# bcgsc/RNA-Bloom

Hardware: AMD Instinct MI355X
Metric: k-mers/sec hashed+inserted into Bloom dBG (k=25, 50M 150bp reads) (higher is better)
Workload: dtype u64

## Files before the change

rna-bloom_amd/csrc/rb_capi.hip:

```cpp
#include <math.h>
#include <stdarg.h>
#include <stdlib.h>
#include <string.h>
#include <time.h>

#include <algorithm>
#include <new>
#include <vector>

#include <functional>
#include <string>
#include <thread>

#include <fcntl.h>
#include <unistd.h>
#include <zlib.h>

#include "rb_pipeline.hpp"

using namespace rb;

namespace {

__global__ void k_popcount_bits(const uint32_t *__restrict__ w, size_t n_words, unsigned long long *out) {
// ... 62 lines not shown

}

extern "C" {

int rb_version(void) { return 1; }
const char *rb_last_error(void) { return rb::last_error_text(); }

int rb_graph_create(const rb_graph_params *p, rb_graph **out) {
    rb_graph *g = nullptr;
    int rc = guarded([&] {
        RB_REQUIRE(p && out, "rb_graph_create: null argument");
        RB_REQUIRE(p->k >= 1 && p->k <= RB_MAX_K, "rb_graph_create: k=%d out of range [1,%d]", p->k, RB_MAX_K);
        RB_REQUIRE(p->dbgbf_bits > 0 && p->cbf_bytes > 0, "rb_graph_create: filter sizes must be positive");
        RB_REQUIRE(p->dbgbf_num_hash >= 1 && p->dbgbf_num_hash <= RB_MAX_HASH && p->cbf_num_hash >= 1 &&
                   p->cbf_num_hash <= RB_MAX_HASH, "rb_graph_create: numHash out of range [1,%d]", RB_MAX_HASH);
        if (p->use_read_paired_kmers)
            RB_REQUIRE(p->pkbf_bits > 0 && p->pkbf_num_hash >= 1 && p->pkbf_num_hash <= RB_MAX_HASH,
                       "rb_graph_create: pair filter parameters invalid");
        int ndev = 0;
        RB_HIP(hipGetDeviceCount(&ndev));
        RB_REQUIRE(p->device >= 0 && p->device < ndev, "rb_graph_create: device %d not present (%d devices)", p->device, ndev);
        RB_HIP(hipSetDevice(p->device));
        g = new rb_graph();
        g->p = *p;
        g->k = p->k;
        g->stranded = p->stranded != 0;
        g->H = std::max(p->dbgbf_num_hash, p->cbf_num_hash);
        g->max_batch_kmers = p->max_batch_kmers > 0 ? p->max_batch_kmers : ((int64_t)1 << 30);
        RB_REQUIRE(p->group_bits >= 0 && p->group_bits <= 64, "rb_graph_create: group_bits out of range [0,64]");
        if (p->group_bits) g->sort_begin_bit = 64 - p->group_bits;
        if (const char *e = getenv("RB_LIGHT_OPS")) g->light_ops = (uint32_t)std::max(1, atoi(e));
        if (const char *e = getenv("RB_SMALL_COMPONENT_OPS")) g->small_ops = (uint32_t)std::max(1, atoi(e));
        if (const char *e = getenv("RB_SORT_BEGIN_BIT")) g->sort_begin_bit = std::max(0, std::min(63, atoi(e)));
        RB_REQUIRE(g->max_batch_kmers <= ((int64_t)1 << 31), "rb_graph_create: max_batch_kmers above 2^31");
        if (const char *e = getenv("RB_CONSUMER_PRIORITY")) RB_HIP(hipStreamCreateWithPriority(&g->stream.s, hipStreamNonBlocking, atoi(e)));
        else RB_HIP(hipStreamCreateWithFlags(&g->stream.s, hipStreamNonBlocking));
        {
            int lo_p = 0, hi_p = 0;
            RB_HIP(hipDeviceGetStreamPriorityRange(&lo_p, &hi_p));
            int pr = hi_p;
            if (const char *e = getenv("RB_PRODUCER_PRIORITY")) pr = atoi(e);
            RB_HIP(hipStreamCreateWithPriority(&g->stream2.s, hipStreamNonBlocking, pr));
            RB_HIP(hipStreamCreateWithPriority(&g->stream3.s, hipStreamNonBlocking, pr));
        }
        RB_HIP(hipStreamCreateWithFlags(&g->pk_stream.s, hipStreamNonBlocking));
        RB_HIP(hipEventCreate(&g->ev0.e));
        RB_HIP(hipEventCreate(&g->ev1.e));
        RB_HIP(hipEventCreateWithFlags(&g->ev2.e, hipEventDisableTiming));
        RB_HIP(hipEventCreateWithFlags(&g->ev3.e, hipEventDisableTiming));
        alloc_bits(g->dbg, p->dbgbf_bits, p->dbgbf_num_hash, 0, p->dbgbf_bits);
        g->cbf_size = p->cbf_bytes; g->cbf_lo = 0; g->cbf_hi = p->cbf_bytes;
        g->cbf_alloc = (((size_t)p->cbf_bytes + 3) / 4 + 1) * 4;
        g->cbf_h = p->cbf_num_hash;
        g->cbf_mod = make_mod((uint64_t)p->cbf_bytes);
        g->cbf = static_cast<uint8_t *>(rb::alloc_best_placed(g->cbf_alloc, "cbf"));
        if (p->use_read_paired_kmers) { alloc_bits(g->rpk, p->pkbf_bits, p->pkbf_num_hash, 0, p->pkbf_bits); alloc_pair_seen(g->rpk); }
        {
            const char *e = getenv("RB_NPF");
            uint32_t l2 = log2_ceil((uint64_t)std::max<int64_t>(p->cbf_bytes / 64, 1));
            l2 = std::max(16u, std::min(28u, l2));
            if (e) l2 = (uint32_t)atoi(e);
            if (l2 >= 8 && l2 <= 30) {
                g->npf.reserve(sizeof(uint64_t) << l2);
                RB_HIP(hipMemset(g->npf.p, 0, sizeof(uint64_t) << l2));
                g->npf_log2 = l2;
// ... 813 lines not shown
```

rna-bloom_amd/csrc/rb_graph.hip:

```cpp
#include <math.h>
#include <stdarg.h>
#include <stdlib.h>
#include <string.h>
#include <time.h>

#include <algorithm>
#include <new>
#include <vector>

#include <functional>
#include <string>
#include <thread>

#include <fcntl.h>
#include <unistd.h>
#include <zlib.h>

#include "rb_pipeline.hpp"

using namespace rb;

namespace rb {
static thread_local char g_err[768] = "";
const char *last_error_text() { return g_err; }
// ... 482 lines not shown
    uint64_t idx[RB_MAX_HASH];
    bool conflict = (st & ST_FOREIGN) != 0;
    for (int j = 0; j < fv.cbf_h; ++j) {
        idx[j] = index_of(multi_hash(h0, (uint32_t)j, fv.kmul), fv.cbf_mod);
        if (n_foreign && !conflict) {
            const uint64_t b = slot_of(idx[j], csf_log2);
            if (!csf || ((csf[b >> 5] >> (uint32_t)(b & 31u)) & 1u)) conflict = table_find(cs, cs_log2, idx[j]) != nullptr;
        }
    }
    if (ops == 0) {
        for (int j = 0; j < fv.cbf_h; ++j) cbf_release(fv.cbf, idx[j]);
        return;
    }
    if (conflict) { status[d] = st | RUN_CONFLICT; return; }
    if (ops > LIGHT_OPS) { status[d] = st | RUN_HEAVY; return; }
    apply_light_run(fv, h0, occ_d, idx, cv_d, 0u, kfirst, krest, tz, start_d + m - ops, ops, mode);
}

__global__ void k_conf_release(FilterView fv, const uint64_t *__restrict__ uniq, const uint32_t *__restrict__ conf_kmers,
                               uint32_t n_conf) {
    uint32_t i = blockIdx.x * blockDim.x + threadIdx.x;
    if (i >= n_conf) return;
    const uint64_t h0 = uniq[conf_kmers[i]];
    for (int j = 0; j < fv.cbf_h; ++j) cbf_release(fv.cbf, index_of(multi_hash(h0, (uint32_t)j, fv.kmul), fv.cbf_mod));
}

__global__ void k_conf_offsets(const uint32_t *__restrict__ conf_kmers, const uint32_t *__restrict__ nops,
                               uint32_t n_conf, uint32_t *__restrict__ sizes) {
    uint32_t i = blockIdx.x * blockDim.x + threadIdx.x;
    if (i < n_conf) sizes[i] = nops[conf_kmers[i]];
    if (i == n_conf) sizes[i] = 0;
}
__global__ void k_label_init(FilterView fv, const uint64_t *__restrict__ uniq, const uint32_t *__restrict__ conf_kmers, uint32_t n_conf,
                             const Slot *ctable, uint32_t c_log2, uint32_t *__restrict__ label, uint32_t *__restrict__ lslot) {
    uint32_t i = blockIdx.x * blockDim.x + threadIdx.x;
    if (i >= n_conf) return;
    const uint32_t d = conf_kmers[i];
    label[d] = d;
    const uint64_t h0 = uniq[d];
    for (int j = 0; j < fv.cbf_h; ++j) {
        const Slot *sl = table_find(ctable, c_log2, index_of(multi_hash(h0, (uint32_t)j, fv.kmul), fv.cbf_mod));
        lslot[(size_t)i * fv.cbf_h + j] = sl ? (uint32_t)(sl - ctable) : CS_NONE;
    }
}
__global__ void k_label_round(int h, const uint32_t *__restrict__ conf_kmers, uint32_t n_conf, Slot *ctable, const uint32_t *__restrict__ lslot,
                              uint32_t *__restrict__ label, uint32_t *__restrict__ changed) {
    uint32_t i = blockIdx.x * blockDim.x + threadIdx.x;
    if (i >= n_conf) return;
    const uint32_t d = conf_kmers[i];
    const uint32_t l0 = __hip_atomic_load(&label[d], __ATOMIC_RELAXED, __HIP_MEMORY_SCOPE_AGENT);
    uint32_t l = l0, sl[RB_MAX_HASH];
    for (int j = 0; j < h; ++j) {
        sl[j] = lslot[(size_t)i * h + j];
        if (sl[j] == CS_NONE) continue;
        const uint32_t v = __hip_atomic_load(reinterpret_cast<const uint32_t *>(&ctable[sl[j]].val), __ATOMIC_RELAXED, __HIP_MEMORY_SCOPE_AGENT);
        l = v < l ? v : l;
    }
    const uint32_t up = __hip_atomic_load(&label[l], __ATOMIC_RELAXED, __HIP_MEMORY_SCOPE_AGENT);
    l = up < l ? up : l;
    bool moved = l != l0;
    if (moved) __hip_atomic_store(&label[d], l, __ATOMIC_RELAXED, __HIP_MEMORY_SCOPE_AGENT);
    for (int j = 0; j < h; ++j)
        if (sl[j] != CS_NONE && atomicMin(reinterpret_cast<uint32_t *>(&ctable[sl[j]].val), l) > l) moved = true;
    if (moved) *changed = 1u;
}
__global__ void k_conf_kmer_keys(const uint32_t *__restrict__ conf_kmers, const uint32_t *__restrict__ label,
                                 uint32_t n_conf, uint64_t *__restrict__ keys) {
    uint32_t i = blockIdx.x * blockDim.x + threadIdx.x;
    if (i < n_conf) { uint32_t d = conf_kmers[i]; keys[i] = ((uint64_t)label[d] << 32) | d; }
}
__global__ void k_conf_expand(const uint32_t *__restrict__ conf_kmers, const uint32_t *__restrict__ conf_off,
                              const uint32_t *__restrict__ counts, const uint32_t *__restrict__ starts,
                              const uint32_t *__restrict__ vals, const uint32_t *__restrict__ status,
                              const uint32_t *__restrict__ nops, const uint32_t *__restrict__ label, uint32_t n_conf,
                              uint64_t *__restrict__ op_key, uint32_t *__restrict__ op_val) {
    const uint32_t wave = (blockIdx.x * blockDim.x + threadIdx.x) >> 3, lane = threadIdx.x & 7u;
    if (wave >= n_conf) return;
    const uint32_t d = conf_kmers[wave];
    const uint32_t ops = nops[d], st = status[d];
    const uint64_t hi = (uint64_t)label[d] << 32;
    const uint32_t base = starts[d] + counts[d] - ops, out = conf_off[wave];
    for (uint32_t i = lane; i < ops; i += 8u) {
        op_key[out + i] = hi | vals[base + i];
        uint32_t kind = i == 0 ? (st >> 12) & 3u : (st >> 14) & 3u;
        op_val[out + i] = d | (kind << 30);
    }
}

__device__ __forceinline__ uint32_t lower_bound_u64(const uint64_t *a, uint32_t n, uint64_t key) {
    uint32_t lo = 0, hi = n;
    while (lo < hi) { uint32_t mid = (lo + hi) >> 1; if (a[mid] < key) lo = mid + 1; else hi = mid; }
    return lo;
}
__device__ void replay_serial(const FilterView &fv, const uint64_t *__restrict__ uniq, const uint64_t *__restrict__ op_key,
                              const uint32_t *__restrict__ op_val, uint32_t os, uint32_t oe) {
    uint64_t idx[RB_MAX_HASH];
    uint32_t c[RB_MAX_HASH], cur_d = 0xFFFFFFFFu;
    for (uint32_t i = os; i < oe; ++i) {
        const uint32_t v = (uint32_t)op_key[i];
        const uint32_t ov = op_val[i], d = ov & 0x3FFFFFFFu, kind = ov >> 30;
        if (d != cur_d) {
            const uint64_t h0 = uniq[d];
            for (int j = 0; j < fv.cbf_h; ++j) {
                idx[j] = index_of(multi_hash(h0, (uint32_t)j, fv.kmul), fv.cbf_mod);
                c[j] = *(volatile uint8_t *)&fv.cbf[idx[j]];
            }
            cur_d = d;
        }
        uint32_t c0[RB_MAX_HASH];
        for (int j = 0; j < fv.cbf_h; ++j) c0[j] = c[j];
        uint32_t mn = c[0];
        for (int j = 1; j < fv.cbf_h; ++j) mn = c[j] < mn ? c[j] : mn;
        cbf_step(c, fv.cbf_h, kind, (mn >= 16u && mn < 127u) ? occ_rnd(fv, v) : 0u);
        for (int j = 0; j < fv.cbf_h; ++j)
            if (c[j] != c0[j]) *(volatile uint8_t *)&fv.cbf[idx[j]] = (uint8_t)c[j];
    }
}
constexpr uint32_t MAX_COMPONENT_KMERS = 8;
__global__ void k_conf_replay_small(FilterView fv, const uint64_t *__restrict__ uniq, const uint64_t *__restrict__ kmer_keys,
                                    uint32_t n_conf, const uint64_t *__restrict__ op_key, const uint32_t *__restrict__ op_val,
                                    uint32_t n_ops, uint32_t *__restrict__ big_list, uint32_t *__restrict__ n_big, int store_cache,
                                    const uint32_t *__restrict__ starts, const uint32_t *__restrict__ vals, uint32_t small_ops) {
    uint32_t i = blockIdx.x * blockDim.x + threadIdx.x;
    if (i >= n_conf) return;
    const uint32_t lab = (uint32_t)(kmer_keys[i] >> 32);
    if (i > 0 && (uint32_t)(kmer_keys[i - 1] >> 32) == lab) return;
    const uint32_t os = lower_bound_u64(op_key, n_ops, (uint64_t)lab << 32);
    const uint32_t oe = lower_bound_u64(op_key, n_ops, ((uint64_t)lab + 1ull) << 32);
    if (oe - os > small_ops) { big_list[atomicAdd(n_big, 1u)] = i; return; }
    replay_serial(fv, uniq, op_key, op_val, os, oe);
    if (store_cache && cache_on(fv))
        for (uint32_t q = i; q < n_conf && (uint32_t)(kmer_keys[q] >> 32) == lab; ++q) {
            const uint32_t dq = (uint32_t)kmer_keys[q];
            const uint64_t h0 = uniq[dq];
            uint32_t mn = 255u;
            for (int j = 0; j < fv.cbf_h; ++j) {
                const uint32_t c = *(volatile uint8_t *)&fv.cbf[index_of(multi_hash(h0, (uint32_t)j, fv.kmul), fv.cbf_mod)];
                mn = c < mn ? c : mn;
            }
            if (mn >= 16u && mn < 128u) cache_store(fv, h0, vals[starts[dq]], cache_exp(mn));
        }
}
__global__ void __launch_bounds__(64) k_conf_replay_big(FilterView fv, const uint64_t *__restrict__ uniq,
                                    const uint64_t *__restrict__ kmer_keys, uint32_t n_conf,
                                    const uint64_t *__restrict__ op_key, const uint32_t *__restrict__ op_val, uint32_t n_ops,
                                    const uint32_t *__restrict__ big_list, const uint32_t *__restrict__ n_big,
                                    uint32_t *__restrict__ dbg, int store_cache,
                                    const uint32_t *__restrict__ starts, const uint32_t *__restrict__ vals) {
    __shared__ uint32_t s_drun[MAX_COMPONENT_KMERS];
    __shared__ uint64_t s_idx[MAX_COMPONENT_KMERS * RB_MAX_HASH];
    __shared__ uint32_t s_val[MAX_COMPONENT_KMERS * RB_MAX_HASH];
    __shared__ uint32_t s_val0[MAX_COMPONENT_KMERS * RB_MAX_HASH];
    __shared__ uint32_t s_slot[MAX_COMPONENT_KMERS][RB_MAX_HASH];
    __shared__ uint64_t s_h0[MAX_COMPONENT_KMERS];
    __shared__ uint32_t s_nu, s_nk;
    const uint32_t lane = threadIdx.x;
    const int H = fv.cbf_h;
    for (uint32_t bi = blockIdx.x; bi < *n_big; bi += gridDim.x) {
        const uint32_t i0 = big_list[bi];
        const uint32_t lab = (uint32_t)(kmer_keys[i0] >> 32);
        const uint32_t i1 = lower_bound_u64(kmer_keys, n_conf, ((uint64_t)lab + 1ull) << 32);
        const uint32_t os = lower_bound_u64(op_key, n_ops, (uint64_t)lab << 32);
        const uint32_t oe = lower_bound_u64(op_key, n_ops, ((uint64_t)lab + 1ull) << 32);
        __syncthreads();
        if (lane == 0) s_nk = 0;
        __syncthreads();
        bool overflow = false;
        for (uint32_t rb0 = i0; rb0 < i1 && !overflow; rb0 += 64u) {
            const bool have = rb0 + lane < i1;
            const uint32_t myd = have ? (uint32_t)kmer_keys[rb0 + lane] : 0u;
            const uint64_t h = have ? uniq[myd] : 0ull;
            unsigned long long pending = __ballot(have);
            while (pending) {
                const int leader = __ffsll((long long)pending) - 1;
                const uint64_t hl = __shfl(h, leader, 64);
                const uint32_t dl = __shfl(myd, leader, 64);
                pending &= ~__ballot(have && h == hl);
                uint32_t q = 0, nkc = s_nk;
                while (q < nkc && s_h0[q] != hl) ++q;
                if (q == nkc) {
                    if (nkc == MAX_COMPONENT_KMERS) { overflow = true; break; }
                    __syncthreads();
                    if (lane == 0) { s_h0[nkc] = hl; s_drun[nkc] = dl; s_nk = nkc + 1u; }
                    __syncthreads();
                }
            }
        }
        if (dbg && lane == 0) { atomicMax(&dbg[1], oe - os); atomicMax(&dbg[2], i1 - i0); atomicAdd(&dbg[3], oe - os); }
        if (overflow) {
            if (dbg && lane == 0) { atomicAdd(&dbg[0], 1u); atomicAdd(&dbg[4], oe - os); }
            if (lane == 0) replay_serial(fv, uniq, op_key, op_val, os, oe);
            continue;
        }
        const uint32_t nk = s_nk;
        __syncthreads();
        if (lane == 0) {
            uint32_t nu = 0;
            for (uint32_t q = 0; q < nk; ++q) {
                const uint64_t h0 = s_h0[q];
                for (int j = 0; j < H; ++j) {
                    const uint64_t idx = index_of(multi_hash(h0, (uint32_t)j, fv.kmul), fv.cbf_mod);
                    uint32_t u = 0;
                    while (u < nu && s_idx[u] != idx) ++u;
                    if (u == nu) { s_idx[u] = idx; s_val0[u] = s_val[u] = fv.cbf[idx]; ++nu; }
                    s_slot[q][j] = u;
                }
            }
            s_nu = nu;
        }
        __syncthreads();
        for (uint32_t base = os; base < oe; base += 64u) {
            const uint32_t i = base + lane;
            uint32_t q = 0, kind = 0, rnd = 0;
            const bool live = i < oe;
            if (live) {
                const uint32_t ov = op_val[i];
                const uint64_t h = uniq[ov & 0x3FFFFFFFu];
                kind = ov >> 30;
                while (q < nk && s_h0[q] != h) ++q;
                rnd = occ_rnd(fv, (uint32_t)op_key[i]);
            }
            uint32_t cursor = 0;
            while (cursor < 64u) {
                bool changes = false;
                if (live && lane >= cursor) {
                    uint32_t mn = s_val[s_slot[q][0]];
                    for (int j = 1; j < H; ++j) { uint32_t c = s_val[s_slot[q][j]]; mn = c < mn ? c : mn; }
                    const bool gate = !((kind == K_INC_IF_POS && mn == 0u) || (kind == K_INC_IF_ZERO && mn != 0u));
                    changes = gate && minifloat_inc(mn, rnd) != mn;
                }
                const unsigned long long win = __ballot(changes);
                if (!win) break;
                const uint32_t first = (uint32_t)__ffsll((long long)win) - 1u;
                if (lane == first) {
                    uint32_t mn = s_val[s_slot[q][0]];
                    for (int j = 1; j < H; ++j) { uint32_t c = s_val[s_slot[q][j]]; mn = c < mn ? c : mn; }
                    for (int j = 0; j < H; ++j) if (s_val[s_slot[q][j]] == mn) s_val[s_slot[q][j]] = mn + 1u;
                }
                __syncthreads();
                cursor = first + 1u;
            }
            __syncthreads();
        }
        if (lane < s_nu && s_val[lane] != s_val0[lane]) fv.cbf[s_idx[lane]] = (uint8_t)s_val[lane];
        if (store_cache && cache_on(fv) && lane < nk) {
            uint32_t mn = s_val[s_slot[lane][0]];
            for (int j = 1; j < H; ++j) { const uint32_t c = s_val[s_slot[lane][j]]; mn = c < mn ? c : mn; }
            if (mn >= 16u && mn < 128u) cache_store(fv, s_h0[lane], vals[starts[s_drun[lane]]], cache_exp(mn));
        }
        __syncthreads();
    }
}

__device__ __forceinline__ uint32_t next_unusable(const uint32_t *__restrict__ vw, uint32_t p, uint32_t L) {
    while (p < L) {
        const uint32_t w = ~vw[p >> 5] >> (p & 31u);
        if (w) { const uint32_t q = p + (uint32_t)__ffs((int)w) - 1u; return q < L ? q : L; }
        p = (p | 31u) + 1u;
    }
    return L;
}
template <int MODE, bool OUT>
__global__ void k_pairs_insert(const uint64_t *__restrict__ codes, const uint32_t *__restrict__ valid,
                               const uint32_t *__restrict__ word_read, const uint32_t *__restrict__ woff,
                               const uint32_t *__restrict__ len, int64_t w0, int64_t nw, int k, int dist,
                               uint32_t *bits, Mod mod, int num_hash, uint64_t kmul,
                               unsigned long long *__restrict__ n_pairs,
                               const uint32_t *__restrict__ chunk_off, uint64_t *__restrict__ out_idx,
                               uint32_t wpr_uniform) {
    int64_t t = (int64_t)blockIdx.x * blockDim.x + threadIdx.x;
    if (t >= nw) return;
    int64_t i = t;
    if (wpr_uniform) { const int64_t nreads = nw / wpr_uniform; i = (t % nreads) * wpr_uniform + t / nreads; }
    const int64_t w = w0 + i;
    const uint32_t r = word_read[w], wr = woff[r], L = len[r];
    const uint32_t b0 = (uint32_t)(w - wr) * 32u;
// ... 708 lines not shown
        uint32_t *conf2 = g->kk1.as<uint32_t>();
        hipLaunchKernelGGL(k_list_compact, dim3(blocks_for(nc0)), dim3(TPB), 0, s, cand, ordered, pos_o, nc0, conf2);
        hipLaunchKernelGGL(k_list_compact, dim3(blocks_for(nc0)), dim3(TPB), 0, s, cand, heavy2, pos_h, nc0, heavy2_list);
        uint32_t n2[2] = {0, 0};
        RB_HIP(hipMemcpyAsync(&n2[0], pos_o + nc0, 4, hipMemcpyDeviceToHost, s));
        RB_HIP(hipMemcpyAsync(&n2[1], pos_h + nc0, 4, hipMemcpyDeviceToHost, s));
        RB_HIP(hipStreamSynchronize(s));
        if (n2[0]) RB_HIP(hipMemcpyAsync(g->confk.p, conf2, (size_t)n2[0] * 4, hipMemcpyDeviceToDevice, s));
        if (n2[1]) {
            RB_HIP(hipMemcpyAsync(changed + 12, &n2[1], 4, hipMemcpyHostToDevice, s));
            hipLaunchKernelGGL(k_cbf_heavy, dim3(std::min<uint32_t>(n2[1], 262144u)), dim3(64), 0, s, fv, uniq, counts, starts,
                               vals, status, nops, g->cvals.as<uint64_t>(), g->tz().as<uint8_t>(), heavy2_list, changed + 12, (uint64_t *)nullptr);
        }
        hc[1] = n2[0];
        g->prof_end("conflict_set");
    }
    release();
    if (hc[0]) {
        g->prof_begin();
        hipLaunchKernelGGL(k_cbf_heavy, dim3(std::min<uint32_t>(hc[0], 262144u)), dim3(64), 0, s, fv, uniq, counts, starts,
                           vals, status, nops, g->cvals.as<uint64_t>(), g->tz().as<uint8_t>(), g->heavy.as<uint32_t>(), ctr, (uint64_t *)nullptr);
        g->prof_end("cbf_heavy");
    }
    if (hc[1]) {
        const uint32_t nck = hc[1];
        g->prof_begin();
        g->conf_sizes.reserve(((size_t)nck + 1) * 4); g->conf_off.reserve(((size_t)nck + 1) * 4);
        hipLaunchKernelGGL(k_conf_offsets, dim3(blocks_for(nck + 1)), dim3(TPB), 0, s, g->confk.as<uint32_t>(), nops, nck, g->conf_sizes.as<uint32_t>());
        g->temp.reserve(scan_temp_bytes((size_t)nck + 1));
        exclusive_scan_u32(g->temp.p, g->temp.cap, g->conf_sizes.as<uint32_t>(), g->conf_off.as<uint32_t>(), (size_t)nck + 1, s);
        uint32_t nco = 0;
        RB_HIP(hipMemcpyAsync(&nco, g->conf_off.as<uint32_t>() + nck, 4, hipMemcpyDeviceToHost, s));
        RB_HIP(hipStreamSynchronize(s));
        g->opk0.reserve((size_t)nco * 8); g->opk1.reserve((size_t)nco * 8);
        g->opv0.reserve((size_t)nco * 4); g->opv1.reserve((size_t)nco * 4);
        g->label.reserve((size_t)D * 4); g->kk0.reserve((size_t)nck * 8); g->kk1.reserve((size_t)nck * 8);
        g->biglist.reserve((size_t)nck * 4);
        const uint32_t *confk = g->confk.as<uint32_t>();
        uint32_t *label = g->label.as<uint32_t>();
        hipLaunchKernelGGL(k_conf_release, dim3(blocks_for(nck)), dim3(TPB), 0, s, fv, uniq, confk, nck);
        g->opk1.reserve(std::max((size_t)nco * 8, (size_t)nck * fv.cbf_h * 4));
        uint32_t *lslot = g->opk1.as<uint32_t>();
        hipLaunchKernelGGL(k_label_init, dim3(blocks_for(nck)), dim3(TPB), 0, s, fv, uniq, confk, nck, g->ctable.as<Slot>(), c_log2, label, lslot);
        const int per_look = nck >= (1u << 20) ? 1 : 2;
        for (int it = 0;; ++it) {
            RB_REQUIRE(it < 100000, "component labelling did not converge");
            uint32_t *flag = ctr + 900 + (it & 31);
            if ((it & 31) == 0) RB_HIP(hipMemsetAsync(ctr + 900, 0, 128, s));
            for (int q = 0; q < per_look; ++q)
                hipLaunchKernelGGL(k_label_round, dim3(blocks_for(nck)), dim3(TPB), 0, s, (int)fv.cbf_h, confk, nck, g->ctable.as<Slot>(), lslot, label, flag);
            uint32_t changed = 0;
            RB_HIP(hipMemcpyAsync(&changed, flag, 4, hipMemcpyDeviceToHost, s));
            RB_HIP(hipStreamSynchronize(s));
            if (!changed) break;
        }
        g->prof_end("conflict_components");
        g->prof_begin();
        hipLaunchKernelGGL(k_conf_kmer_keys, dim3(blocks_for(nck)), dim3(TPB), 0, s, confk, label, nck, g->kk0.as<uint64_t>());
        g->temp.reserve(std::max(sort_pairs_temp_bytes(nco), sort_keys_temp_bytes(nck)));
        hipLaunchKernelGGL(k_conf_expand, dim3(blocks_for((int64_t)nck * 8)), dim3(TPB), 0, s, confk, g->conf_off.as<uint32_t>(),
                           counts, starts, vals, status, nops, label, nck, g->opk0.as<uint64_t>(), g->opv0.as<uint32_t>());
        const int label_end = 32 + (int)std::max(1u, log2_ceil((uint64_t)D));
        sort_keys_u64(g->temp.p, g->temp.cap, g->kk0.as<uint64_t>(), g->kk1.as<uint64_t>(), nck, 32, label_end, s);
        sort_pairs_u64_u32_2r(g->temp.p, g->temp.cap, g->opk0.as<uint64_t>(), g->opk1.as<uint64_t>(),
                              g->opv0.as<uint32_t>(), g->opv1.as<uint32_t>(), nco, 0, (int)std::min(32u, std::max(1u, g->occ_bits)), 32, label_end, s);
        g->prof_end("conflict_gather_sort");
        g->prof_begin();
        RB_HIP(hipMemsetAsync(ctr + 4, 0, 4, s));
        hipLaunchKernelGGL(k_conf_replay_small, dim3(blocks_for(nck)), dim3(TPB), 0, s, fv, uniq, g->kk1.as<uint64_t>(), nck,
                           g->opk1.as<uint64_t>(), g->opv1.as<uint32_t>(), nco, g->biglist.as<uint32_t>(), ctr + 4, (int)(mode != M_COUNT_ONLY), starts, vals, g->small_ops);
        hipLaunchKernelGGL(k_conf_replay_big, dim3(std::min<uint32_t>(nck, 262144u)), dim3(64), 0, s, fv, uniq, g->kk1.as<uint64_t>(), nck,
                           g->opk1.as<uint64_t>(), g->opv1.as<uint32_t>(), nco, g->biglist.as<uint32_t>(), ctr + 4,
                           getenv("RB_DEBUG") ? ctr + 600 : (uint32_t *)nullptr, (int)(mode != M_COUNT_ONLY), starts, vals);
        g->prof_end("conflict_replay");
        if (getenv("RB_DEBUG")) {
            uint32_t nb = 0;
            RB_HIP(hipMemcpy(&nb, ctr + 4, 4, hipMemcpyDeviceToHost));
            uint32_t dv[5];
            RB_HIP(hipMemcpy(dv, ctr + 600, 20, hipMemcpyDeviceToHost));
            fprintf(stderr, "[rb] N=%zu D=%u heavy=%u conflict_runs=%u conflict_ops=%u big_components=%u n_foreign=%u | big: serial_fallback=%u (ops %u) max_ops=%u max_runs=%u ops_in_big=%u\n", N, D, hc[0], nck, nco, nb, n_foreign, dv[0], dv[4], dv[1], dv[2], dv[3]);
        }
        if (stats) stats->conflict_ops += nco;
    }
    RB_HIP(hipGetLastError());
}

}
void rb::add_range(rb_graph *g, const rb_batch *b, int64_t first, int64_t n, unsigned flags, rb_add_stats *stats) {
    RB_REQUIRE(!g->shard, "rb_graph_add_batch: this handle is one shard of a distributed graph; drive it with the rb_shard_* phases");
    RB_REQUIRE(b->device == g->p.device, "batch lives on device %d, graph on %d", b->device, g->p.device);
    RB_REQUIRE(first >= 0 && n >= 0 && first + n <= b->n_reads, "rb_graph_add_batch: bad read range");
    RB_HIP(hipSetDevice(g->p.device));
    hipStream_t s = g->stream;
    const int mode_hash = g->stranded ? ((flags & RB_ADD_REVCOMP) ? 2 : 0) : 1;
    const int mode = (flags & RB_ADD_COUNT_IF_PRESENT) ? M_COUNT_IF_PRESENT : M_ADD;
    const bool pairs = (flags & RB_ADD_STORE_READ_PAIRS) != 0;
    if (pairs) RB_REQUIRE(g->rpk.bits && g->read_d > 0, "STORE_READ_PAIRS needs use_read_paired_kmers and a read pair distance > 0");
    const uint32_t max_pos = b->max_len >= (uint32_t)g->k ? b->max_len - (uint32_t)g->k : 0u;
    uint32_t pos_bits = 1;
    while ((1u << pos_bits) <= max_pos && pos_bits < 31) ++pos_bits;
    const int64_t max_reads = ((int64_t)1 << (32 - pos_bits)) - 1;
    const bool wide_off = getenv("RB_WIDE_PREFILTER") && atoi(getenv("RB_WIDE_PREFILTER")) == 0;
    const bool npf_path = g->npf_log2 && (g->k <= 31 || (g->k <= 64 && !wide_off));
    const int wmul = getenv("RB_WINDOW_MUL") ? std::max(1, atoi(getenv("RB_WINDOW_MUL"))) : 3;
    const int64_t max_words = std::max<int64_t>(std::min<int64_t>((npf_path ? wmul : 1) * g->max_batch_kmers, (int64_t)7 << 29) / 32, 1);
    const auto &wo = b->h_woff;
    struct Sub { int64_t r0, r1, w0, nw; uint32_t N; int64_t total; };
    const bool use_npf = npf_path && (mode == M_ADD || mode == M_COUNT_IF_PRESENT);
    g->use_mpf = use_npf && g->mpf_log2b && !getenv("RB_NO_MPF") && (uint32_t)g->k >= g->mpf_m &&
                 (g->k <= RB_MPF_MAX_K ? (uint32_t)g->k - g->mpf_m + 1u <= RB_MPF_MAX_RING
                                       : filter_wide_mpf_ok(b, b->h_woff.empty() ? 0 : (int64_t)b->h_woff[(size_t)(first + n)] - (int64_t)b->h_woff[(size_t)first], g->k));
    g->seq_codes = b->codes; g->seq_woff = b->woff; g->seq_wpr = b->wpr_uniform;
    struct MpfScope { rb_graph *g; ~MpfScope() { g->use_mpf = false; g->seq_codes = nullptr; g->seq_woff = nullptr; g->seq_wpr = 0; g->occ_bits = 32; } } mpf_scope{g};
// ... 194 lines not shown
```

rna-bloom_amd/csrc/rb_pipeline.hpp:

```cpp
#pragma once
#include <string.h>

#include <algorithm>
#include <condition_variable>
#include <mutex>
#include <new>
#include <shared_mutex>
#include <functional>
#include <memory>
#include <string>
#include <thread>
#include <vector>

#include "rb_internal.hpp"
#include "rb_kernels.hpp"

namespace rb {

constexpr int TPB = 256;
constexpr size_t DEVCTR_BYTES = 4096;
inline unsigned blocks_for(int64_t n, int tpb = TPB) { return (unsigned)((n + tpb - 1) / tpb); }

struct BitFilter {
    uint32_t *bits = nullptr;
// ... 259 lines not shown
struct rb_trav;
using rb::BitFilter; using rb::FilterView; using rb::Mod; using rb::DevBuf; using rb::kmul_of;
struct rb_query_ctx {
    rb::Stream st;
    rb::DevBuf b0, b1, b2, b3;
};
struct rb_graph {
    ~rb_graph();
    std::shared_mutex rw;
    std::mutex qm;
    std::condition_variable qcv;
    std::vector<std::unique_ptr<rb_query_ctx>> qfree;
    int qmade = 0;
    static constexpr int kMaxQueryCtx = 32;
    int shard_rank = 0, shard_count = 1;
    ShardState *shard = nullptr;
    rb_trav *trav = nullptr;
    rb_graph_params p{};
    int k = 0, H = 0;
    bool stranded = false;
    BitFilter dbg, rpk, fpk;
    uint8_t *cbf = nullptr;
    int64_t cbf_size = 0;
    int64_t cbf_lo = 0, cbf_hi = 0;
    size_t cbf_alloc = 0;
    Mod cbf_mod{1, 0, 0};
    int cbf_h = 0;
    int read_d = -1, frag_d = -1;
    uint64_t ordinal = 0;
    int64_t max_batch_kmers = 0;
    int sort_begin_bit = 28;
    uint32_t light_ops = 96;
    uint32_t small_ops = 32;
    rb::Stream stream;
    rb::Stream stream2;
    rb::Stream stream3;
    rb::Stream pk_stream;
    rb::Event ev0, ev1, ev2, ev3;
    DevPool ingest_pool;
    struct GroupSlot { DevBuf keys1, valsT, vals1, tz, uniq, counts, starts, brun, bnr ; uint32_t sweep_T = 0, n_main = 0; size_t N = 0; uint32_t D = 0; int flags = 0; uint32_t live = 0; int bucket_target = 0;  };
    GroupSlot slots[2];
    int cur = 0;
    DevBuf &keys1() { return slots[cur].keys1; }
    DevBuf &vals1() { return slots[cur].vals1; }
    DevBuf &tz() { return slots[cur].tz; }
    DevBuf &uniq() { return slots[cur].uniq; }
    DevBuf &counts() { return slots[cur].counts; }
    DevBuf &starts() { return slots[cur].starts; }
    DevBuf temp2, devctr2, pairs_ctr;
    DevBuf sw_st, sw_temp;
    int pf_streak = 0, pf_skip_left = 0;
    float last_present_frac = 0.0f;
    DevBuf npf, chunk_mask, npf_tot, wstate;
    uint32_t npf_log2 = 0;
    DevBuf mpf;
    uint32_t mpf_log2b = 0, mpf_m = 0;
    const uint64_t *seq_codes = nullptr;
    const uint32_t *seq_woff = nullptr;
    uint32_t seq_wpr = 0;
    uint32_t seq_first = 0;
    uint64_t *group_in_keys = nullptr;
    uint32_t *group_in_vals = nullptr;
    uint32_t occ_bits = 32;
    bool use_mpf = false;
    DevBuf chunk_cnt, chunk_off, keys0, vals0, status, nops, temp,
        ftable, ctable, heavy, confk, conf_sizes, conf_off, opk0, opk1, opv0, opv1, label, kk0, kk1, biglist, cvals, foreign, devctr, qbuf0, qbuf1, qbuf2, qbuf3,
// ... 152 lines not shown
```

Measured before the change: 42.67 billion.

## Replace conflict op gather-sort with per-component k-way merge of sorted runs

Conflict replay used to expand every conflicting k-mer's ops into a global array and radix-sort it by label and value. Component replay now merges each component's already-sorted per-k-mer runs directly, serially per thread for small components and wave-cooperatively for big ones up to a run limit. The expand and sort path only runs when some component exceeds that limit, which the labelling rounds detect by counting runs per label. The intent is to drop a large sort and its buffers from the hot path, at the cost of extra shared memory, more complex merge kernels and an atomic count in every labelling round.

```diff
diff --git a/rna-bloom_amd/csrc/rb_capi.hip b/rna-bloom_amd/csrc/rb_capi.hip
--- a/rna-bloom_amd/csrc/rb_capi.hip
+++ b/rna-bloom_amd/csrc/rb_capi.hip
@@ -118,6 +118,7 @@
         if (p->group_bits) g->sort_begin_bit = 64 - p->group_bits;
         if (const char *e = getenv("RB_LIGHT_OPS")) g->light_ops = (uint32_t)std::max(1, atoi(e));
         if (const char *e = getenv("RB_SMALL_COMPONENT_OPS")) g->small_ops = (uint32_t)std::max(1, atoi(e));
+        if (const char *e = getenv("RB_MERGE_COMPONENT_RUNS")) g->merge_runs = (uint32_t)std::min(256, std::max(0, atoi(e)));
         if (const char *e = getenv("RB_SORT_BEGIN_BIT")) g->sort_begin_bit = std::max(0, std::min(63, atoi(e)));
         RB_REQUIRE(g->max_batch_kmers <= ((int64_t)1 << 31), "rb_graph_create: max_batch_kmers above 2^31");
         if (const char *e = getenv("RB_CONSUMER_PRIORITY")) RB_HIP(hipStreamCreateWithPriority(&g->stream.s, hipStreamNonBlocking, atoi(e)));
diff --git a/rna-bloom_amd/csrc/rb_graph.hip b/rna-bloom_amd/csrc/rb_graph.hip
--- a/rna-bloom_amd/csrc/rb_graph.hip
+++ b/rna-bloom_amd/csrc/rb_graph.hip
@@ -538,11 +538,13 @@
     if (i == n_conf) sizes[i] = 0;
 }
 __global__ void k_label_init(FilterView fv, const uint64_t *__restrict__ uniq, const uint32_t *__restrict__ conf_kmers, uint32_t n_conf,
-                             const Slot *ctable, uint32_t c_log2, uint32_t *__restrict__ label, uint32_t *__restrict__ lslot) {
+                             const Slot *ctable, uint32_t c_log2, uint32_t *__restrict__ label, uint32_t *__restrict__ lslot,
+                             uint32_t *__restrict__ lcnt0, uint32_t *__restrict__ lcnt1) {
     uint32_t i = blockIdx.x * blockDim.x + threadIdx.x;
     if (i >= n_conf) return;
     const uint32_t d = conf_kmers[i];
     label[d] = d;
+    lcnt0[d] = 0u; lcnt1[d] = 0u;
     const uint64_t h0 = uniq[d];
     for (int j = 0; j < fv.cbf_h; ++j) {
         const Slot *sl = table_find(ctable, c_log2, index_of(multi_hash(h0, (uint32_t)j, fv.kmul), fv.cbf_mod));
@@ -550,7 +552,8 @@
     }
 }
 __global__ void k_label_round(int h, const uint32_t *__restrict__ conf_kmers, uint32_t n_conf, Slot *ctable, const uint32_t *__restrict__ lslot,
-                              uint32_t *__restrict__ label, uint32_t *__restrict__ changed) {
+                              uint32_t *__restrict__ label, uint32_t *__restrict__ changed, uint32_t *__restrict__ lcnt_cur,
+                              uint32_t *__restrict__ lcnt_next, uint32_t merge_runs) {
     uint32_t i = blockIdx.x * blockDim.x + threadIdx.x;
     if (i >= n_conf) return;
     const uint32_t d = conf_kmers[i];
@@ -569,11 +572,21 @@
     for (int j = 0; j < h; ++j)
         if (sl[j] != CS_NONE && atomicMin(reinterpret_cast<uint32_t *>(&ctable[sl[j]].val), l) > l) moved = true;
     if (moved) *changed = 1u;
+    if (lcnt_cur) {
+        lcnt_next[d] = 0u;
+        if (atomicAdd(&lcnt_cur[l], 1u) >= merge_runs) changed[1] = 1u;
+    }
 }
 __global__ void k_conf_kmer_keys(const uint32_t *__restrict__ conf_kmers, const uint32_t *__restrict__ label,
                                  uint32_t n_conf, uint64_t *__restrict__ keys) {
     uint32_t i = blockIdx.x * blockDim.x + threadIdx.x;
     if (i < n_conf) { uint32_t d = conf_kmers[i]; keys[i] = ((uint64_t)label[d] << 32) | d; }
+}
+__global__ void k_conf_over_sizes(const uint32_t *__restrict__ conf_kmers, const uint32_t *__restrict__ nops, const uint32_t *__restrict__ label,
+                                  const uint32_t *__restrict__ lcnt, uint32_t merge_runs, uint32_t n_conf, uint32_t *__restrict__ sizes) {
+    uint32_t i = blockIdx.x * blockDim.x + threadIdx.x;
+    if (i < n_conf) { const uint32_t d = conf_kmers[i]; sizes[i] = lcnt[label[d]] > merge_runs ? nops[d] : 0u; }
+    if (i == n_conf) sizes[i] = 0;
 }
 __global__ void k_conf_expand(const uint32_t *__restrict__ conf_kmers, const uint32_t *__restrict__ conf_off,
                               const uint32_t *__restrict__ counts, const uint32_t *__restrict__ starts,
@@ -582,10 +595,12 @@
                               uint64_t *__restrict__ op_key, uint32_t *__restrict__ op_val) {
     const uint32_t wave = (blockIdx.x * blockDim.x + threadIdx.x) >> 3, lane = threadIdx.x & 7u;
     if (wave >= n_conf) return;
+    const uint32_t out = conf_off[wave];
+    if (conf_off[wave + 1] == out) return;
     const uint32_t d = conf_kmers[wave];
     const uint32_t ops = nops[d], st = status[d];
     const uint64_t hi = (uint64_t)label[d] << 32;
-    const uint32_t base = starts[d] + counts[d] - ops, out = conf_off[wave];
+    const uint32_t base = starts[d] + counts[d] - ops;
     for (uint32_t i = lane; i < ops; i += 8u) {
         op_key[out + i] = hi | vals[base + i];
         uint32_t kind = i == 0 ? (st >> 12) & 3u : (st >> 14) & 3u;
@@ -598,13 +613,10 @@
     while (lo < hi) { uint32_t mid = (lo + hi) >> 1; if (a[mid] < key) lo = mid + 1; else hi = mid; }
     return lo;
 }
-__device__ void replay_serial(const FilterView &fv, const uint64_t *__restrict__ uniq, const uint64_t *__restrict__ op_key,
-                              const uint32_t *__restrict__ op_val, uint32_t os, uint32_t oe) {
+struct SerialReplay {
     uint64_t idx[RB_MAX_HASH];
     uint32_t c[RB_MAX_HASH], cur_d = 0xFFFFFFFFu;
-    for (uint32_t i = os; i < oe; ++i) {
-        const uint32_t v = (uint32_t)op_key[i];
-        const uint32_t ov = op_val[i], d = ov & 0x3FFFFFFFu, kind = ov >> 30;
+    __device__ __forceinline__ void op(const FilterView &fv, const uint64_t *__restrict__ uniq, uint32_t d, uint32_t kind, uint32_t v) {
         if (d != cur_d) {
             const uint64_t h0 = uniq[d];
             for (int j = 0; j < fv.cbf_h; ++j) {
@@ -621,22 +633,51 @@
         for (int j = 0; j < fv.cbf_h; ++j)
             if (c[j] != c0[j]) *(volatile uint8_t *)&fv.cbf[idx[j]] = (uint8_t)c[j];
     }
-}
+};
 constexpr uint32_t MAX_COMPONENT_KMERS = 8;
-__global__ void k_conf_replay_small(FilterView fv, const uint64_t *__restrict__ uniq, const uint64_t *__restrict__ kmer_keys,
-                                    uint32_t n_conf, const uint64_t *__restrict__ op_key, const uint32_t *__restrict__ op_val,
-                                    uint32_t n_ops, uint32_t *__restrict__ big_list, uint32_t *__restrict__ n_big, int store_cache,
-                                    const uint32_t *__restrict__ starts, const uint32_t *__restrict__ vals, uint32_t small_ops) {
-    uint32_t i = blockIdx.x * blockDim.x + threadIdx.x;
+constexpr uint32_t SMALL_MAX_RUNS = 32;
+constexpr uint32_t SMALL_TPB = 64;
+__global__ void __launch_bounds__(SMALL_TPB) k_conf_replay_small(FilterView fv, const uint64_t *__restrict__ uniq, const uint64_t *__restrict__ kmer_keys,
+                                    uint32_t n_conf, const uint32_t *__restrict__ counts, const uint32_t *__restrict__ status,
+                                    const uint32_t *__restrict__ nops, uint32_t *__restrict__ big_list, uint32_t *__restrict__ n_big, int store_cache,
+                                    const uint32_t *__restrict__ starts, const uint32_t *__restrict__ vals, uint32_t small_ops, uint32_t *__restrict__ dbg) {
+    __shared__ uint32_t s_pos[SMALL_MAX_RUNS][SMALL_TPB], s_end[SMALL_MAX_RUNS][SMALL_TPB], s_head[SMALL_MAX_RUNS][SMALL_TPB];
+    const uint32_t t = threadIdx.x;
+    uint32_t i = blockIdx.x * blockDim.x + t;
     if (i >= n_conf) return;
     const uint32_t lab = (uint32_t)(kmer_keys[i] >> 32);
     if (i > 0 && (uint32_t)(kmer_keys[i - 1] >> 32) == lab) return;
-    const uint32_t os = lower_bound_u64(op_key, n_ops, (uint64_t)lab << 32);
-    const uint32_t oe = lower_bound_u64(op_key, n_ops, ((uint64_t)lab + 1ull) << 32);
-    if (oe - os > small_ops) { big_list[atomicAdd(n_big, 1u)] = i; return; }
-    replay_serial(fv, uniq, op_key, op_val, os, oe);
+    uint32_t nr = 0, no = 0;
+    bool big = false;
+    for (uint32_t q = i; q < n_conf && (uint32_t)(kmer_keys[q] >> 32) == lab; ++q) {
+        if (nr == SMALL_MAX_RUNS) { big = true; break; }
+        const uint32_t d = (uint32_t)kmer_keys[q], ops = nops[d];
+        no += ops;
+        if (no > small_ops) { big = true; break; }
+        const uint32_t base = starts[d] + counts[d] - ops;
+        s_pos[nr][t] = base; s_end[nr][t] = base + ops; s_head[nr][t] = vals[base];
+        ++nr;
+    }
+    if (big) { big_list[atomicAdd(n_big, 1u)] = i; return; }
+    if (dbg) atomicAdd(&dbg[6], 1u);
+    uint32_t live = nr == 32u ? 0xFFFFFFFFu : (1u << nr) - 1u, fresh = live;
+    uint32_t cur_r = 0xFFFFFFFFu, cur_d = 0, cur_st = 0;
+    SerialReplay R;
+    while (live) {
+        uint32_t m = live, r = (uint32_t)__ffs((int)m) - 1u, h = s_head[r][t];
+        for (m &= m - 1u; m; m &= m - 1u) {
+            const uint32_t r2 = (uint32_t)__ffs((int)m) - 1u, h2 = s_head[r2][t];
+            if (h2 < h) { h = h2; r = r2; }
+        }
+        if (r != cur_r) { cur_r = r; cur_d = (uint32_t)kmer_keys[i + r]; cur_st = status[cur_d]; }
+        R.op(fv, uniq, cur_d, ((fresh >> r) & 1u) ? (cur_st >> 12) & 3u : (cur_st >> 14) & 3u, h);
+        fresh &= ~(1u << r);
+        const uint32_t p = s_pos[r][t] + 1u;
+        if (p == s_end[r][t]) live &= ~(1u << r);
+        else { s_pos[r][t] = p; s_head[r][t] = vals[p]; }
+    }
     if (store_cache && cache_on(fv))
-        for (uint32_t q = i; q < n_conf && (uint32_t)(kmer_keys[q] >> 32) == lab; ++q) {
+        for (uint32_t q = i; q < i + nr; ++q) {
             const uint32_t dq = (uint32_t)kmer_keys[q];
             const uint64_t h0 = uniq[dq];
             uint32_t mn = 255u;
@@ -647,12 +688,21 @@
             if (mn >= 16u && mn < 128u) cache_store(fv, h0, vals[starts[dq]], cache_exp(mn));
         }
 }
+constexpr uint32_t MERGE_MAX_RUNS = 256, MERGE_W = MERGE_MAX_RUNS / 64;
+constexpr uint64_t MERGE_DONE = 1ull << 32;
+__device__ __forceinline__ uint64_t wave_min_u64(uint64_t v) {
+    for (int o = 32; o; o >>= 1) { const uint64_t x = __shfl_xor(v, o, 64); v = x < v ? x : v; }
+    return v;
+}
+template <bool MERGE>
 __global__ void __launch_bounds__(64) k_conf_replay_big(FilterView fv, const uint64_t *__restrict__ uniq,
                                     const uint64_t *__restrict__ kmer_keys, uint32_t n_conf,
-                                    const uint64_t *__restrict__ op_key, const uint32_t *__restrict__ op_val, uint32_t n_ops,
+                                    const uint64_t *__restrict__ op_key, const uint32_t *__restrict__ op_val, const uint32_t *__restrict__ n_ops_p,
                                     const uint32_t *__restrict__ big_list, const uint32_t *__restrict__ n_big,
                                     uint32_t *__restrict__ dbg, int store_cache,
-                                    const uint32_t *__restrict__ starts, const uint32_t *__restrict__ vals) {
+                                    const uint32_t *__restrict__ starts, const uint32_t *__restrict__ vals,
+                                    const uint32_t *__restrict__ counts, const uint32_t *__restrict__ status, const uint32_t *__restrict__ nops,
+                                    uint32_t merge_runs) {
     __shared__ uint32_t s_drun[MAX_COMPONENT_KMERS];
     __shared__ uint64_t s_idx[MAX_COMPONENT_KMERS * RB_MAX_HASH];
     __shared__ uint32_t s_val[MAX_COMPONENT_KMERS * RB_MAX_HASH];
@@ -660,14 +710,39 @@
     __shared__ uint32_t s_slot[MAX_COMPONENT_KMERS][RB_MAX_HASH];
     __shared__ uint64_t s_h0[MAX_COMPONENT_KMERS];
     __shared__ uint32_t s_nu, s_nk;
+    __shared__ uint32_t s_cocc[64], s_cval[64];
     const uint32_t lane = threadIdx.x;
     const int H = fv.cbf_h;
+    const uint32_t n_ops = MERGE ? 0u : *n_ops_p;
     for (uint32_t bi = blockIdx.x; bi < *n_big; bi += gridDim.x) {
         const uint32_t i0 = big_list[bi];
         const uint32_t lab = (uint32_t)(kmer_keys[i0] >> 32);
         const uint32_t i1 = lower_bound_u64(kmer_keys, n_conf, ((uint64_t)lab + 1ull) << 32);
-        const uint32_t os = lower_bound_u64(op_key, n_ops, (uint64_t)lab << 32);
-        const uint32_t oe = lower_bound_u64(op_key, n_ops, ((uint64_t)lab + 1ull) << 32);
+        if ((i1 - i0 > merge_runs) == MERGE) continue;
+        uint32_t os = 0, oe = 0;
+        uint32_t c_pos[MERGE_W], c_end[MERGE_W], c_dk[MERGE_W];
+        uint32_t c_st[MERGE_W];
+        uint64_t c_head[MERGE_W];
+        if (MERGE) {
+            uint32_t tot = 0;
+#pragma unroll
+            for (uint32_t w = 0; w < MERGE_W; ++w) {
+                const uint32_t r = i0 + lane + 64u * w;
+                c_pos[w] = c_end[w] = 0; c_dk[w] = 0; c_st[w] = 0; c_head[w] = MERGE_DONE;
+                if (r < i1) {
+                    const uint32_t d = (uint32_t)kmer_keys[r], ops = nops[d], st = status[d];
+                    c_pos[w] = starts[d] + counts[d] - ops; c_end[w] = c_pos[w] + ops;
+                    c_dk[w] = d; c_st[w] = ((st >> 12) & 15u) | 16u;
+                    c_head[w] = vals[c_pos[w]];
+                    tot += ops;
+                }
+            }
+            for (int o = 32; o; o >>= 1) tot += __shfl_xor(tot, o, 64);
+            oe = tot;
+        } else {
+            os = lower_bound_u64(op_key, n_ops, (uint64_t)lab << 32);
+            oe = lower_bound_u64(op_key, n_ops, ((uint64_t)lab + 1ull) << 32);
+        }
         __syncthreads();
         if (lane == 0) s_nk = 0;
         __syncthreads();
@@ -692,15 +767,17 @@
                 }
             }
         }
-        if (dbg && lane == 0) { atomicMax(&dbg[1], oe - os); atomicMax(&dbg[2], i1 - i0); atomicAdd(&dbg[3], oe - os); }
+        if (dbg && lane == 0) { atomicMax(&dbg[1], oe - os); atomicMax(&dbg[2], i1 - i0); atomicAdd(&dbg[3], oe - os); if (MERGE) atomicAdd(&dbg[5], 1u); }
         if (overflow) {
             if (dbg && lane == 0) { atomicAdd(&dbg[0], 1u); atomicAdd(&dbg[4], oe - os); }
-            if (lane == 0) replay_serial(fv, uniq, op_key, op_val, os, oe);
-            continue;
+            if (!MERGE) {
+                if (lane == 0) { SerialReplay R; for (uint32_t i = os; i < oe; ++i) R.op(fv, uniq, op_val[i] & 0x3FFFFFFFu, op_val[i] >> 30, (uint32_t)op_key[i]); }
+                continue;
+            }
         }
         const uint32_t nk = s_nk;
         __syncthreads();
-        if (lane == 0) {
+        if (lane == 0 && !overflow) {
             uint32_t nu = 0;
             for (uint32_t q = 0; q < nk; ++q) {
                 const uint64_t h0 = s_h0[q];
@@ -715,16 +792,66 @@
             s_nu = nu;
         }
         __syncthreads();
-        for (uint32_t base = os; base < oe; base += 64u) {
-            const uint32_t i = base + lane;
+        SerialReplay R;
+        for (uint32_t base = os;; base += 64u) {
+            uint32_t n_chunk;
+            if (MERGE) {
+                n_chunk = 0;
+                while (n_chunk < 64u) {
+                    uint64_t h1 = MERGE_DONE, h2 = MERGE_DONE;
+                    uint32_t w1 = 0;
+#pragma unroll
+                    for (uint32_t w = 0; w < MERGE_W; ++w) {
+                        if (c_head[w] < h1) { h2 = h1; h1 = c_head[w]; w1 = w; }
+                        else if (c_head[w] < h2) h2 = c_head[w];
+                    }
+                    const uint64_t m1 = wave_min_u64(h1);
+                    if (m1 == MERGE_DONE) break;
+                    const uint32_t owner = (uint32_t)__ffsll((long long)__ballot(h1 == m1)) - 1u;
+                    const uint64_t m2 = wave_min_u64(lane == owner ? h2 : h1);
+                    uint32_t po = 0, en = 0, dd = 0, kk = 0;
+#pragma unroll
+                    for (uint32_t w = 0; w < MERGE_W; ++w)
+                        if (w == w1) { po = c_pos[w]; en = c_end[w]; dd = c_dk[w]; kk = c_st[w]; }
+                    po = __shfl(po, (int)owner, 64); en = __shfl(en, (int)owner, 64);
+                    dd = __shfl(dd, (int)owner, 64); kk = __shfl(kk, (int)owner, 64);
+                    const uint32_t ip = po + lane;
+                    const bool in = ip < en && lane < 64u - n_chunk;
+                    const uint32_t v = in ? vals[ip] : 0u;
+                    const unsigned long long take = __ballot(in && (uint64_t)v < m2);
+                    const uint32_t len = ~take ? (uint32_t)__ffsll((long long)~take) - 1u : 64u;
+                    if (lane < len) {
+                        s_cocc[n_chunk + lane] = v;
+                        s_cval[n_chunk + lane] = dd | (((lane == 0 && (kk & 16u)) ? kk & 3u : (kk >> 2) & 3u) << 30);
+                    }
+                    if (lane == owner) {
+#pragma unroll
+                        for (uint32_t w = 0; w < MERGE_W; ++w)
+                            if (w == w1) {
+                                c_pos[w] = po + len; c_st[w] = kk & 15u;
+                                c_head[w] = c_pos[w] < c_end[w] ? (uint64_t)vals[c_pos[w]] : MERGE_DONE;
+                            }
+                    }
+                    n_chunk += len;
+                }
+                __syncthreads();
+            } else {
+                n_chunk = base < oe ? (oe - base < 64u ? oe - base : 64u) : 0u;
+            }
+            if (!n_chunk) break;
+            if (MERGE && overflow) {
+                if (lane == 0) for (uint32_t i = 0; i < n_chunk; ++i) R.op(fv, uniq, s_cval[i] & 0x3FFFFFFFu, s_cval[i] >> 30, s_cocc[i]);
+                __syncthreads();
+                continue;
+            }
             uint32_t q = 0, kind = 0, rnd = 0;
-            const bool live = i < oe;
+            const bool live = lane < n_chunk;
             if (live) {
-                const uint32_t ov = op_val[i];
+                const uint32_t ov = MERGE ? s_cval[lane] : op_val[base + lane];
                 const uint64_t h = uniq[ov & 0x3FFFFFFFu];
                 kind = ov >> 30;
                 while (q < nk && s_h0[q] != h) ++q;
-                rnd = occ_rnd(fv, (uint32_t)op_key[i]);
+                rnd = occ_rnd(fv, MERGE ? s_cocc[lane] : (uint32_t)op_key[base + lane]);
             }
             uint32_t cursor = 0;
             while (cursor < 64u) {
@@ -748,6 +875,7 @@
             }
             __syncthreads();
         }
+        if (overflow) continue;
         if (lane < s_nu && s_val[lane] != s_val0[lane]) fv.cbf[s_idx[lane]] = (uint8_t)s_val[lane];
         if (store_cache && cache_on(fv) && lane < nk) {
             uint32_t mn = s_val[s_slot[lane][0]];
@@ -1522,53 +1650,75 @@
         uint32_t nco = 0;
         RB_HIP(hipMemcpyAsync(&nco, g->conf_off.as<uint32_t>() + nck, 4, hipMemcpyDeviceToHost, s));
         RB_HIP(hipStreamSynchronize(s));
-        g->opk0.reserve((size_t)nco * 8); g->opk1.reserve((size_t)nco * 8);
-        g->opv0.reserve((size_t)nco * 4); g->opv1.reserve((size_t)nco * 4);
         g->label.reserve((size_t)D * 4); g->kk0.reserve((size_t)nck * 8); g->kk1.reserve((size_t)nck * 8);
         g->biglist.reserve((size_t)nck * 4);
         const uint32_t *confk = g->confk.as<uint32_t>();
         uint32_t *label = g->label.as<uint32_t>();
         hipLaunchKernelGGL(k_conf_release, dim3(blocks_for(nck)), dim3(TPB), 0, s, fv, uniq, confk, nck);
-        g->opk1.reserve(std::max((size_t)nco * 8, (size_t)nck * fv.cbf_h * 4));
+        g->opk1.reserve((size_t)nck * fv.cbf_h * 4);
         uint32_t *lslot = g->opk1.as<uint32_t>();
-        hipLaunchKernelGGL(k_label_init, dim3(blocks_for(nck)), dim3(TPB), 0, s, fv, uniq, confk, nck, g->ctable.as<Slot>(), c_log2, label, lslot);
+        uint32_t *lcnt[2] = {g->cvals.as<uint32_t>(), g->cvals.as<uint32_t>() + D};
+        const uint32_t merge_runs = g->merge_runs;
+        hipLaunchKernelGGL(k_label_init, dim3(blocks_for(nck)), dim3(TPB), 0, s, fv, uniq, confk, nck, g->ctable.as<Slot>(), c_log2, label, lslot, lcnt[0], lcnt[1]);
         const int per_look = nck >= (1u << 20) ? 1 : 2;
+        uint32_t look[2] = {0, 0};
+        const uint32_t *lcnt_final = lcnt[0];
         for (int it = 0;; ++it) {
             RB_REQUIRE(it < 100000, "component labelling did not converge");
-            uint32_t *flag = ctr + 900 + (it & 31);
-            if ((it & 31) == 0) RB_HIP(hipMemsetAsync(ctr + 900, 0, 128, s));
-            for (int q = 0; q < per_look; ++q)
-                hipLaunchKernelGGL(k_label_round, dim3(blocks_for(nck)), dim3(TPB), 0, s, (int)fv.cbf_h, confk, nck, g->ctable.as<Slot>(), lslot, label, flag);
-            uint32_t changed = 0;
-            RB_HIP(hipMemcpyAsync(&changed, flag, 4, hipMemcpyDeviceToHost, s));
+            uint32_t *flag = ctr + 960 + 2 * (it & 15);
+            if ((it & 15) == 0) RB_HIP(hipMemsetAsync(ctr + 960, 0, 128, s));
+            for (int q = 0; q < per_look; ++q) {
+                const bool last = q == per_look - 1;
+                hipLaunchKernelGGL(k_label_round, dim3(blocks_for(nck)), dim3(TPB), 0, s, (int)fv.cbf_h, confk, nck, g->ctable.as<Slot>(), lslot, label, flag,
+                                   last ? lcnt[it & 1] : (uint32_t *)nullptr, lcnt[(it + 1) & 1], merge_runs);
+            }
+            RB_HIP(hipMemcpyAsync(look, flag, 8, hipMemcpyDeviceToHost, s));
             RB_HIP(hipStreamSynchronize(s));
-            if (!changed) break;
-        }
+            lcnt_final = lcnt[it & 1];
+            if (!look[0]) break;
+        }
+        const bool oversize = look[1] != 0;
         g->prof_end("conflict_components");
         g->prof_begin();
         hipLaunchKernelGGL(k_conf_kmer_keys, dim3(blocks_for(nck)), dim3(TPB), 0, s, confk, label, nck, g->kk0.as<uint64_t>());
-        g->temp.reserve(std::max(sort_pairs_temp_bytes(nco), sort_keys_temp_bytes(nck)));
-        hipLaunchKernelGGL(k_conf_expand, dim3(blocks_for((int64_t)nck * 8)), dim3(TPB), 0, s, confk, g->conf_off.as<uint32_t>(),
-                           counts, starts, vals, status, nops, label, nck, g->opk0.as<uint64_t>(), g->opv0.as<uint32_t>());
+        g->temp.reserve(sort_keys_temp_bytes(nck));
         const int label_end = 32 + (int)std::max(1u, log2_ceil((uint64_t)D));
         sort_keys_u64(g->temp.p, g->temp.cap, g->kk0.as<uint64_t>(), g->kk1.as<uint64_t>(), nck, 32, label_end, s);
-        sort_pairs_u64_u32_2r(g->temp.p, g->temp.cap, g->opk0.as<uint64_t>(), g->opk1.as<uint64_t>(),
-                              g->opv0.as<uint32_t>(), g->opv1.as<uint32_t>(), nco, 0, (int)std::min(32u, std::max(1u, g->occ_bits)), 32, label_end, s);
+        if (oversize) {
+            uint32_t *over_off = g->conf_off.as<uint32_t>();
+            hipLaunchKernelGGL(k_conf_over_sizes, dim3(blocks_for(nck + 1)), dim3(TPB), 0, s, confk, nops, label, lcnt_final, merge_runs, nck, g->conf_sizes.as<uint32_t>());
+            exclusive_scan_u32(g->temp.p, g->temp.cap, g->conf_sizes.as<uint32_t>(), over_off, (size_t)nck + 1, s);
+            uint32_t n_over = 0;
+            RB_HIP(hipMemcpyAsync(&n_over, over_off + nck, 4, hipMemcpyDeviceToHost, s));
+            RB_HIP(hipStreamSynchronize(s));
+            g->opk0.reserve((size_t)n_over * 8); g->opk1.reserve((size_t)n_over * 8);
+            g->opv0.reserve((size_t)n_over * 4); g->opv1.reserve((size_t)n_over * 4);
+            g->temp.reserve(sort_pairs_temp_bytes(n_over));
+            hipLaunchKernelGGL(k_conf_expand, dim3(blocks_for((int64_t)nck * 8)), dim3(TPB), 0, s, confk, over_off,
+                               counts, starts, vals, status, nops, label, nck, g->opk0.as<uint64_t>(), g->opv0.as<uint32_t>());
+            sort_pairs_u64_u32_2r(g->temp.p, g->temp.cap, g->opk0.as<uint64_t>(), g->opk1.as<uint64_t>(),
+                                  g->opv0.as<uint32_t>(), g->opv1.as<uint32_t>(), n_over, 0, (int)std::min(32u, std::max(1u, g->occ_bits)), 32, label_end, s);
+        }
         g->prof_end("conflict_gather_sort");
         g->prof_begin();
         RB_HIP(hipMemsetAsync(ctr + 4, 0, 4, s));
-        hipLaunchKernelGGL(k_conf_replay_small, dim3(blocks_for(nck)), dim3(TPB), 0, s, fv, uniq, g->kk1.as<uint64_t>(), nck,
-                           g->opk1.as<uint64_t>(), g->opv1.as<uint32_t>(), nco, g->biglist.as<uint32_t>(), ctr + 4, (int)(mode != M_COUNT_ONLY), starts, vals, g->small_ops);
-        hipLaunchKernelGGL(k_conf_replay_big, dim3(std::min<uint32_t>(nck, 262144u)), dim3(64), 0, s, fv, uniq, g->kk1.as<uint64_t>(), nck,
-                           g->opk1.as<uint64_t>(), g->opv1.as<uint32_t>(), nco, g->biglist.as<uint32_t>(), ctr + 4,
-                           getenv("RB_DEBUG") ? ctr + 600 : (uint32_t *)nullptr, (int)(mode != M_COUNT_ONLY), starts, vals);
+        uint32_t *dbg = getenv("RB_DEBUG") ? ctr + 600 : (uint32_t *)nullptr;
+        hipLaunchKernelGGL(k_conf_replay_small, dim3(blocks_for(nck, (int)SMALL_TPB)), dim3(SMALL_TPB), 0, s, fv, uniq, g->kk1.as<uint64_t>(), nck,
+                           counts, status, nops, g->biglist.as<uint32_t>(), ctr + 4, (int)(mode != M_COUNT_ONLY), starts, vals, g->small_ops, dbg);
+        hipLaunchKernelGGL(k_conf_replay_big<true>, dim3(std::min<uint32_t>(nck, 262144u)), dim3(64), 0, s, fv, uniq, g->kk1.as<uint64_t>(), nck,
+                           (const uint64_t *)nullptr, (const uint32_t *)nullptr, (const uint32_t *)nullptr, g->biglist.as<uint32_t>(), ctr + 4,
+                           dbg, (int)(mode != M_COUNT_ONLY), starts, vals, counts, status, nops, merge_runs);
+        if (oversize)
+            hipLaunchKernelGGL(k_conf_replay_big<false>, dim3(std::min<uint32_t>(nck, 262144u)), dim3(64), 0, s, fv, uniq, g->kk1.as<uint64_t>(), nck,
+                               g->opk1.as<uint64_t>(), g->opv1.as<uint32_t>(), g->conf_off.as<uint32_t>() + nck, g->biglist.as<uint32_t>(), ctr + 4,
+                               dbg, (int)(mode != M_COUNT_ONLY), starts, vals, counts, status, nops, merge_runs);
         g->prof_end("conflict_replay");
         if (getenv("RB_DEBUG")) {
             uint32_t nb = 0;
             RB_HIP(hipMemcpy(&nb, ctr + 4, 4, hipMemcpyDeviceToHost));
-            uint32_t dv[5];
-            RB_HIP(hipMemcpy(dv, ctr + 600, 20, hipMemcpyDeviceToHost));
-            fprintf(stderr, "[rb] N=%zu D=%u heavy=%u conflict_runs=%u conflict_ops=%u big_components=%u n_foreign=%u | big: serial_fallback=%u (ops %u) max_ops=%u max_runs=%u ops_in_big=%u\n", N, D, hc[0], nck, nco, nb, n_foreign, dv[0], dv[4], dv[1], dv[2], dv[3]);
+            uint32_t dv[7];
+            RB_HIP(hipMemcpy(dv, ctr + 600, 28, hipMemcpyDeviceToHost));
+            fprintf(stderr, "[rb] N=%zu D=%u heavy=%u conflict_runs=%u conflict_ops=%u small_components=%u big_components=%u (merged %u, sorted %u) n_foreign=%u | big: serial_fallback=%u (ops %u) max_ops=%u max_runs=%u ops_in_big=%u\n", N, D, hc[0], nck, nco, dv[6], nb, dv[5], nb - dv[5], n_foreign, dv[0], dv[4], dv[1], dv[2], dv[3]);
         }
         if (stats) stats->conflict_ops += nco;
     }
diff --git a/rna-bloom_amd/csrc/rb_pipeline.hpp b/rna-bloom_amd/csrc/rb_pipeline.hpp
--- a/rna-bloom_amd/csrc/rb_pipeline.hpp
+++ b/rna-bloom_amd/csrc/rb_pipeline.hpp
@@ -315,6 +315,7 @@
     int sort_begin_bit = 28;
     uint32_t light_ops = 96;
     uint32_t small_ops = 32;
+    uint32_t merge_runs = 64;
     rb::Stream stream;
     rb::Stream stream2;
     rb::Stream stream3;
```

After: 42.33 billion. About the same (-0.8%).
